# NIRVANALAN/GaussianAnything

Hardware: NVIDIA H100
Metric: 512^2 views/sec @100k Gaussians (surfel raster fwd+bwd) (higher is better)
Workload: dtype f32

## Files before the change

gaussiananything_b200/csrc/raster_bin.cu:

```cuda
#include "raster_common.cuh"
#include "device_once.cuh"

#define SCAN_THREADS 1024
#define SCAN_TILES_PER_THREAD 8
#define SORT_WARP_MAX 512

__global__ void __launch_bounds__(SCAN_THREADS)
scan_tiles_kernel(RasterDims d, RasterWs ws)
{
    __shared__ uint32_t s_warp[32];
    __shared__ uint32_t s_carry;
    __shared__ int s_big;
    const int n = d.NV * d.T;
    if (threadIdx.x == 0) { s_carry = 0; s_big = 0; }
    __syncthreads();
    const int lane = threadIdx.x & 31, warp = threadIdx.x >> 5;
    const uint4 *cnt4 = reinterpret_cast<const uint4 *>(ws.tile_count);
    for (int base = 0; base < n; base += SCAN_THREADS * SCAN_TILES_PER_THREAD) {
        uint32_t v[SCAN_TILES_PER_THREAD];
#pragma unroll
        for (int j = 0; j < SCAN_TILES_PER_THREAD; j++) {
            const int i = base + j * SCAN_THREADS + threadIdx.x;
            v[j] = 0u;
#pragma unroll
            for (int q = 0; q < GA_TILE_REPLICAS / 4; q++) {
                const uint4 c = i < n ? cnt4[(size_t)i * (GA_TILE_REPLICAS / 4) + q] : make_uint4(0u, 0u, 0u, 0u);
                v[j] += ((c.x + c.y) + c.z) + c.w;
            }
        }
        uint32_t excl[SCAN_TILES_PER_THREAD];
#pragma unroll
        for (int j = 0; j < SCAN_TILES_PER_THREAD; j++) {
            if (base + j * SCAN_THREADS >= n) { excl[j] = 0u; continue; }
            if (v[j] > SORT_WARP_MAX) ws.big_tiles[atomicAdd(&s_big, 1)] = (uint32_t)(base + j * SCAN_THREADS + threadIdx.x);
            uint32_t x = v[j];
#pragma unroll
            for (int o = 1; o < 32; o <<= 1) {
                uint32_t y = __shfl_up_sync(0xffffffffu, x, o);
                if (lane >= o) x += y;
            }
            if (lane == 31) s_warp[warp] = x;
            __syncthreads();
            if (warp == 0) {
                uint32_t wv = s_warp[lane], wx = wv;
#pragma unroll
                for (int o = 1; o < 32; o <<= 1) {
                    uint32_t y = __shfl_up_sync(0xffffffffu, wx, o);
                    if (lane >= o) wx += y;
                }
                s_warp[lane] = wx - wv;
            }
            __syncthreads();
            excl[j] = s_carry + s_warp[warp] + x - v[j];
            __syncthreads();
            if (threadIdx.x == SCAN_THREADS - 1) s_carry = excl[j] + v[j];
            __syncthreads();
        }
#pragma unroll
        for (int j = 0; j < SCAN_TILES_PER_THREAD; j++) {
            const int i = base + j * SCAN_THREADS + threadIdx.x;
            if (i >= n) continue;
            ws.tile_start[i] = excl[j];
            uint32_t run = excl[j];
            uint4 *dst = reinterpret_cast<uint4 *>(ws.tile_count) + (size_t)i * (GA_TILE_REPLICAS / 4);
#pragma unroll
            for (int q = 0; q < GA_TILE_REPLICAS / 4; q++) {
                const uint4 c = cnt4[(size_t)i * (GA_TILE_REPLICAS / 4) + q];
                uint4 cur;
                cur.x = run; run += c.x;
                cur.y = run; run += c.y;
                cur.z = run; run += c.z;
                cur.w = run; run += c.w;
                dst[q] = cur;
            }
        }
    }
    __syncthreads();
    if (threadIdx.x == 0) {
        const uint32_t total = s_carry;
        ws.tile_start[n] = total;
        ws.status[0] = (int32_t)total;
        ws.status[1] = ((int64_t)total > d.max_instances) ? 1 : 0;
        ws.status[3] = s_big;
    }
}

__global__ void __launch_bounds__(256)
scatter_kernel(RasterDims d, RasterWs ws)
{
    const int view = blockIdx.y;
    const int i = blockIdx.x * 256 + threadIdx.x;
    if (i >= d.P || ws.status[1]) return;
    const size_t vi = (size_t)view * d.P + i;
    const uint32_t r = ws.rect[vi];
    if (r == 0) return;
    const int x0 = r & 255, y0 = (r >> 8) & 255, x1 = (r >> 16) & 255, y1 = r >> 24;
    const unsigned long long key =
        ((unsigned long long)__float_as_uint(ws.depth[vi]) << 32) | (unsigned long long)(uint32_t)i;
    const int rep = (threadIdx.x >> 5) & (GA_TILE_REPLICAS - 1);
    for (int y = y0; y < y1; y++)
        for (int x = x0; x < x1; x++) {
            const size_t t = (size_t)view * d.T + y * d.gx + x;
            const uint32_t slot = atomicAdd(&ws.tile_count[t * GA_TILE_REPLICAS + rep], 1u);
            ws.keys[slot] = key;
        }
}

__device__ __forceinline__ void block_bitonic_sort(unsigned long long *a, int n)
{
    int n2 = 1;
    while (n2 < n) n2 <<= 1;
    for (int k = 2; k <= n2; k <<= 1) {
        for (int t = threadIdx.x; t < n2 / 2; t += blockDim.x) {
            const int blk = t / (k / 2), off = t % (k / 2);
            const int i = blk * k + off, p = blk * k + k - 1 - off;
            if (p < n) {
                unsigned long long x = a[i], y = a[p];
                if (x > y) { a[i] = y; a[p] = x; }
            }
        }
        __syncthreads();
        for (int j = k / 4; j >= 1; j >>= 1) {
            for (int t = threadIdx.x; t < n2 / 2; t += blockDim.x) {
                const int i = (t / j) * 2 * j + (t % j), p = i + j;
                if (p < n) {
                    unsigned long long x = a[i], y = a[p];
                    if (x > y) { a[i] = y; a[p] = x; }
                }
            }
            __syncthreads();
        }
    }
}

#define SORT_SMEM_KEYS 4096

template <int KPL>
__device__ __forceinline__ void warp_shuffle_stages(unsigned long long (&v)[KPL], int lane, int k, int jstart)
{
#pragma unroll 1
    for (int j = jstart; j >= 1; j >>= 1) {
        const bool lower = (lane & j) == 0;
#pragma unroll
        for (int r = 0; r < KPL; r++) {
            const bool asc = ((((r << 5) | lane) & k) == 0);
            const unsigned long long mine = v[r];
            const unsigned long long other = __shfl_xor_sync(0xffffffffu, mine, j);
            const bool keep_min = (lower == asc);
            v[r] = keep_min ? (mine < other ? mine : other) : (mine > other ? mine : other);
        }
    }
}

template <int KPL>
__device__ __forceinline__ void warp_bitonic_sort(unsigned long long (&v)[KPL], int lane)
{
    constexpr int N = 32 * KPL;
#pragma unroll 1
    for (int k = 2; k <= 32; k <<= 1) warp_shuffle_stages<KPL>(v, lane, k, k >> 1);
#pragma unroll
    for (int k = 64; k <= N; k <<= 1) {
#pragma unroll
        for (int j = k >> 1; j >= 32; j >>= 1) {
            const int jr = j >> 5;
#pragma unroll
            for (int r = 0; r < KPL; r++) {
                if ((r & jr) == 0) {
                    const bool asc = (((r << 5) & k) == 0);
                    unsigned long long a = v[r], b = v[r | jr];
                    const bool sw = asc ? (a > b) : (a < b);
                    v[r] = sw ? b : a;
                    v[r | jr] = sw ? a : b;
                }
            }
        }
        warp_shuffle_stages<KPL>(v, lane, k, 16);
    }
}

template <int KPL>
__device__ __forceinline__ void warp_sort_tile(unsigned long long *gk, uint32_t *gid, int n, int lane)
{
    unsigned long long v[KPL];
#pragma unroll
    for (int r = 0; r < KPL; r++) {
        const int i = r * 32 + lane;
        v[r] = i < n ? gk[i] : 0xffffffffffffffffull;
    }
    warp_bitonic_sort<KPL>(v, lane);
#pragma unroll
    for (int r = 0; r < KPL; r++) {
        const int i = r * 32 + lane;
        if (i < n) {
            gk[i] = v[r];
            gid[i] = (uint32_t)(v[r] & 0xffffffffull);
        }
    }
}

#define SORT_THREADS 256
__global__ void __launch_bounds__(SORT_THREADS, 3)
sort_tiles_kernel(RasterDims d, RasterWs ws, int big_ctas)
{
    __shared__ unsigned long long s_keys[SORT_SMEM_KEYS];
    if (ws.status[1]) return;
    if ((int)blockIdx.x < big_ctas) {
        const int nbig = ws.status[3];
        for (int b = blockIdx.x; b < nbig; b += big_ctas) {
            const uint32_t t = ws.big_tiles[b];
            const uint32_t start = ws.tile_start[t], end = ws.tile_start[t + 1];
            const int n = (int)(end - start);
            unsigned long long *gk = ws.keys + start;
            if (n <= SORT_SMEM_KEYS) {
                for (int i = threadIdx.x; i < n; i += blockDim.x) s_keys[i] = gk[i];
                __syncthreads();
                block_bitonic_sort(s_keys, n);
                for (int i = threadIdx.x; i < n; i += blockDim.x) {
                    const unsigned long long k = s_keys[i];
                    gk[i] = k;
                    ws.ids[start + i] = (uint32_t)(k & 0xffffffffull);
                }
                __syncthreads();
            } else {
                if (threadIdx.x == 0) atomicAdd(&ws.status[2], 1);
                block_bitonic_sort(gk, n);
                for (int i = threadIdx.x; i < n; i += blockDim.x)
                    ws.ids[start + i] = (uint32_t)(gk[i] & 0xffffffffull);
                __syncthreads();
            }
        }
        return;
    }
    const size_t t = (size_t)(blockIdx.x - big_ctas) * (SORT_THREADS / 32) + (threadIdx.x >> 5);
    if (t >= (size_t)d.NV * d.T) return;
    const int lane = threadIdx.x & 31;
    const uint32_t start = ws.tile_start[t], end = ws.tile_start[t + 1];
    const int n = (int)(end - start);
    if (n == 0 || n > SORT_WARP_MAX) return;
    unsigned long long *gk = ws.keys + start;
    uint32_t *gid = ws.ids + start;
    if (n <= 32) warp_sort_tile<1>(gk, gid, n, lane);
    else if (n <= 128) warp_sort_tile<4>(gk, gid, n, lane);
    else if (n <= 256) warp_sort_tile<8>(gk, gid, n, lane);
    else warp_sort_tile<16>(gk, gid, n, lane);
}

cudaError_t ga_launch_binning(const RasterDims &d, const RasterWs &w, cudaStream_t s, int32_t *status_host,
                              cudaEvent_t status_event)
{
    scan_tiles_kernel<<<1, SCAN_THREADS, 0, s>>>(d, w);
    if (status_host) {
        cudaError_t e = cudaMemcpyAsync(status_host, w.status, 4 * sizeof(int32_t), cudaMemcpyDeviceToHost, s);
        if (e != cudaSuccess) return e;
    }
    if (status_event) {
        cudaError_t e = cudaEventRecord(status_event, s);
        if (e != cudaSuccess) return e;
    }
    dim3 grid((d.P + 255) / 256, d.NV);
    scatter_kernel<<<grid, 256, 0, s>>>(d, w);
    const int tiles = d.NV * d.T;
    const int big_ctas = tiles < ga_sm_count() ? tiles : ga_sm_count();
    sort_tiles_kernel<<<big_ctas + (tiles + SORT_THREADS / 32 - 1) / (SORT_THREADS / 32), SORT_THREADS, 0, s>>>(d, w, big_ctas);
    return cudaGetLastError();
}
```

gaussiananything_b200/csrc/raster_render.cu:

```cuda
#include "raster_common.cuh"
#include "device_once.cuh"

#define CHUNK 256

__device__ __forceinline__ float fast_rcp(float x)
{
    float r;
    asm("rcp.approx.ftz.f32 %0, %1;" : "=f"(r) : "f"(x));
    return r;
}
__device__ __forceinline__ float fast_ex2(float x)
{
    float r;
    asm("ex2.approx.ftz.f32 %0, %1;" : "=f"(r) : "f"(x));
    return r;
}
#define GA_M_C0 (GA_FAR_N / (GA_FAR_N - GA_NEAR_N))
#define GA_M_C1 (GA_FAR_N * GA_NEAR_N / (GA_FAR_N - GA_NEAR_N))
#define GA_NEG_HALF_LOG2E (-0.72134752044448170368f)

struct PixelGeom {
    float s0, s1, p2, rho3d, rho2d, dx, dy, depth, G, alpha;
    bool use3d;
};

__device__ __forceinline__ bool eval_pair(const float4 a, const float4 b, const float4 c,
                                          float pfx, float pfy, PixelGeom &o,
                                          float &k0, float &k1, float &k2,
                                          float &l0, float &l1, float &l2)
{
    k0 = pfx * b.z - a.x; k1 = pfx * b.w - a.y; k2 = pfx * c.x - a.z;
    l0 = pfy * b.z - a.w; l1 = pfy * b.w - b.x; l2 = pfy * c.x - b.y;
    const float p0 = k1 * l2 - k2 * l1, p1 = k2 * l0 - k0 * l2, p2 = k0 * l1 - k1 * l0;
    if (p2 == 0.0f) return false;
    const float ip = fast_rcp(p2);
    o.p2 = p2;
    o.s0 = p0 * ip; o.s1 = p1 * ip;
    o.rho3d = o.s0 * o.s0 + o.s1 * o.s1;
    o.dx = c.y - pfx; o.dy = c.z - pfy;
    o.rho2d = GA_FILTER_INV_SQUARE * (o.dx * o.dx + o.dy * o.dy);
    o.use3d = o.rho3d <= o.rho2d;
    const float rho = fminf(o.rho3d, o.rho2d);
    o.depth = o.use3d ? (o.s0 * b.z + o.s1 * b.w) + c.x : c.x;
    if (o.depth < GA_NEAR_N) return false;
    o.G = fast_ex2(rho * GA_NEG_HALF_LOG2E);
    o.alpha = fminf(0.99f, c.w * o.G);
    return o.alpha >= 1.0f / 255.0f;
}

struct TileBox { int x0, y0, w, h; };
__device__ __forceinline__ TileBox clip_box(const float4 bb, int ox, int oy, int xmax, int ymax)
{
    const float x0 = ceilf(fmaxf(bb.x, (float)ox)), x1 = floorf(fminf(bb.y, (float)xmax));
    const float y0 = ceilf(fmaxf(bb.z, (float)oy)), y1 = floorf(fminf(bb.w, (float)ymax));
    if (!(x1 >= x0 && y1 >= y0)) return {0, 0, 0, 0};
    return {(int)x0 - ox, (int)y0 - oy, (int)(x1 - x0) + 1, (int)(y1 - y0) + 1};
}

#define FWD_PAIRS 4096

struct FwdSmem {
    float4 rec[6][CHUNK];
    float2 pair[FWD_PAIRS];
    uint32_t mask[CHUNK / 32][256];
    int base[CHUNK + 1];
    uint32_t box[CHUNK];
    int cnt[CHUNK];
    int wsum[8];
};

template <bool LISTS>
__global__ void __launch_bounds__(256, 3)
render_fwd_kernel(RasterDims d, RasterWs ws, const float *__restrict__ bg,
                  float *__restrict__ out_color, float *__restrict__ out_allmap)
{
    extern __shared__ __align__(16) uint8_t fwd_smem_raw[];
    FwdSmem &sm = *reinterpret_cast<FwdSmem *>(fwd_smem_raw);
    if (ws.status[1]) return;
    const int view = blockIdx.z;
    const int tile = blockIdx.y * d.gx + blockIdx.x;
    const int warp = threadIdx.x >> 5, lane = threadIdx.x & 31;
    const int ox = blockIdx.x * GA_BLOCK_X, oy = blockIdx.y * GA_BLOCK_Y;
    const int lxi = (warp & 1) * 8 + (lane & 7), lyi = (warp >> 1) * 4 + (lane >> 3);
    const int pix_local = lyi * 16 + lxi;
    const int pxi = ox + lxi, pyi = oy + lyi;
    const bool inside = pxi < d.W && pyi < d.H;
    const float oxf = (float)ox, oyf = (float)oy;

    const uint32_t start = ws.tile_start[(size_t)view * d.T + tile];
    const uint32_t end = ws.tile_start[(size_t)view * d.T + tile + 1];
    const int total = (int)(end - start);
    const float *rec_base = ws.rec + (size_t)view * d.P * GA_REC_F;

    bool done = !inside;
    float T = 1.0f, C0 = 0, C1 = 0, C2 = 0, N0 = 0, N1 = 0, N2 = 0;
    float Dacc = 0, M1 = 0, M2 = 0, dist = 0, median_depth = 0;
    int last_contributor = 0, median_contributor = -1;
    int nl = 0;
    uint4 *my_list = nullptr;
    if (LISTS) my_list = ws.lists + ((size_t)view * d.T + tile) * (size_t)d.list_k * 256 + pix_local;

    for (int c0 = 0; c0 < total; c0 += CHUNK) {
        if (__syncthreads_count(done) == 256) break;
        const int cnt = min(CHUNK, total - c0);
        if (LISTS) sm.cnt[threadIdx.x] = 0;
        int npairs = 0;
        if ((int)threadIdx.x < cnt) {
            const uint32_t id = ws.ids[start + c0 + threadIdx.x];
            const float4 *src = reinterpret_cast<const float4 *>(rec_base + (size_t)id * GA_REC_F);
            const float4 a = __ldg(src), b = __ldg(src + 1), c = __ldg(src + 2);
            const float4 nr = __ldg(src + 3), bb = __ldg(src + 4), gb = __ldg(src + 5);
            const float k0 = oxf * b.z - a.x, k1 = oxf * b.w - a.y, k2 = oxf * c.x - a.z;
            const float l0 = oyf * b.z - a.w, l1 = oyf * b.w - b.x, l2 = oyf * c.x - b.y;
            const float Cx = k1 * l2 - k2 * l1, Cy = k2 * l0 - k0 * l2, Cz = k0 * l1 - k1 * l0;
            const float Ax = b.w * l2 - c.x * l1, Ay = c.x * l0 - b.z * l2, Az = b.z * l1 - b.w * l0;
            const float Bx = k1 * c.x - k2 * b.w, By = k2 * b.z - k0 * c.x, Bz = k0 * b.w - k1 * b.z;
            sm.rec[0][threadIdx.x] = make_float4(Cx, Cy, Cz, Ax);
            sm.rec[1][threadIdx.x] = make_float4(Ay, Az, Bx, By);
            sm.rec[2][threadIdx.x] = make_float4(Bz, b.z, b.w, c.x);
            sm.rec[3][threadIdx.x] = make_float4(c.y - oxf, c.z - oyf, c.w, 0.f);
            sm.rec[4][threadIdx.x] = nr;
            sm.rec[5][threadIdx.x] = gb;
            const TileBox q = clip_box(bb, ox, oy, min(ox + 15, d.W - 1), min(oy + 15, d.H - 1));
            npairs = q.w * q.h;
            sm.box[threadIdx.x] = npairs ? (uint32_t)(q.x0 | q.y0 << 4 | q.w << 8 | (65536 / q.w + 1) << 13) : 0u;
        }
        int incl = npairs;
#pragma unroll
        for (int o = 1; o < 32; o <<= 1) {
            const int y = __shfl_up_sync(0xffffffffu, incl, o);
            if (lane >= o) incl += y;
        }
        if (lane == 31) sm.wsum[warp] = incl;
        __syncthreads();
#pragma unroll
        for (int k = 0; k < 8; k++) incl += k < warp ? sm.wsum[k] : 0;
        sm.base[threadIdx.x] = incl - npairs;
        if (threadIdx.x == CHUNK - 1) sm.base[CHUNK] = incl;

        int t0 = 0, base = 0;
        while (t0 < cnt) {
#pragma unroll
            for (int k = 0; k < CHUNK / 32; k++) sm.mask[k][threadIdx.x] = 0u;
            const int t1 = t0 + __syncthreads_count((int)threadIdx.x >= t0 && (int)threadIdx.x < cnt &&
                                                    incl - base <= FWD_PAIRS);
            const int wpairs = sm.base[t1] - base;
            for (int q = threadIdx.x; q < wpairs; q += 256) {
                const int Q = base + q;
                int jj = t0;
#pragma unroll
                for (int step = CHUNK / 2; step > 0; step >>= 1)
                    if (jj + step < t1 && sm.base[jj + step] <= Q) jj += step;
                const uint32_t bx = sm.box[jj];
                const int k = Q - sm.base[jj], w = (bx >> 8) & 31;
                const int ry = (k * (int)(bx >> 13)) >> 16;
                const int lx = (int)(bx & 15) + k - ry * w, ly = (int)((bx >> 4) & 15) + ry;
                const float dxf = (float)lx, dyf = (float)ly;
                const float4 f0 = sm.rec[0][jj], f1 = sm.rec[1][jj], f2 = sm.rec[2][jj], f3 = sm.rec[3][jj];
                const float p0 = f0.x + dxf * f0.w + dyf * f1.z;
                const float p1 = f0.y + dxf * f1.x + dyf * f1.w;
                const float p2 = f0.z + dxf * f1.y + dyf * f2.x;
                const float ip = fast_rcp(p2);
                const float s0 = p0 * ip, s1 = p1 * ip;
                const float rho3d = s0 * s0 + s1 * s1;
                const float ddx = f3.x - dxf, ddy = f3.y - dyf;
                const float rho2d = GA_FILTER_INV_SQUARE * __fmaf_rn(ddx, ddx, __fmul_rn(ddy, ddy));
                const float rho = fminf(rho3d, rho2d);
                const float depth = (rho3d <= rho2d) ? (s0 * f2.y + s1 * f2.z) + f2.w : f2.w;
                const float alpha = fminf(0.99f, f3.z * fast_ex2(rho * GA_NEG_HALF_LOG2E));
                if (p2 != 0.0f && depth >= GA_NEAR_N && alpha >= 1.0f / 255.0f) {
                    sm.pair[q] = make_float2(alpha, depth);
                    atomicOr(&sm.mask[jj >> 5][ly * 16 + lx], 1u << (jj & 31));
                }
            }
            __syncthreads();
            if (!done) {
                int wi = t0 >> 5;
                const int wlast = (t1 - 1) >> 5;
                uint32_t m = sm.mask[wi][pix_local];
                while (true) {
                    while (m == 0u && wi < wlast) m = sm.mask[++wi][pix_local];
                    if (m == 0u) break;
                    const int jj = wi * 32 + __ffs(m) - 1;
                    m &= m - 1;
                    const uint32_t bx = sm.box[jj];
                    const int k = (lyi - (int)((bx >> 4) & 15)) * (int)((bx >> 8) & 31) + (lxi - (int)(bx & 15));
                    const float2 ad = sm.pair[sm.base[jj] - base + k];
                    const float alpha = ad.x, depth = ad.y;
                    const float test_T = T * (1 - alpha);
                    if (test_T < 0.0001f) { done = true; break; }
                    const float4 nr = sm.rec[4][jj], gb = sm.rec[5][jj];
                    const int contributor = c0 + jj + 1;
                    const float w = alpha * T;
                    const float A = 1 - T;
                    const float mm = GA_M_C0 - GA_M_C1 * fast_rcp(depth);
                    dist += (mm * mm * A + M2 - 2 * mm * M1) * w;
                    Dacc += depth * w;
                    M1 += mm * w;
                    M2 += mm * mm * w;
                    if (T > 0.5f) { median_depth = depth; median_contributor = contributor; }
                    N0 += nr.x * w; N1 += nr.y * w; N2 += nr.z * w;
                    C0 += nr.w * w; C1 += gb.x * w; C2 += gb.y * w;
                    T = test_T;
                    last_contributor = contributor;
                    if (LISTS) {
                        atomicAdd(&sm.cnt[jj], 1);
                        if (nl < d.list_k)
                            my_list[(size_t)nl * 256] = make_uint4((uint32_t)(contributor - 1), __float_as_uint(alpha),
                                                                   __float_as_uint(depth), 0u);
                        nl++;
                    }
                }
            }
            t0 = t1;
            if (t0 < cnt) base = sm.base[t0];
            if (__syncthreads_count(done) == 256) break;
        }
        if (LISTS && (int)threadIdx.x < cnt) ws.inst_cnt[start + c0 + threadIdx.x] = (uint32_t)sm.cnt[threadIdx.x];
    }
    if (LISTS) {
        if (inside) ws.n_list[(size_t)view * d.H * d.W + (size_t)pyi * d.W + pxi] = nl;
        if (nl > d.list_k) ws.tile_flag[(size_t)view * d.T + tile] = 1u;
    }
    if (inside) {
        const size_t HW = (size_t)d.H * d.W;
        const size_t pix = (size_t)pyi * d.W + pxi;
        float *fT = ws.final_T + (size_t)view * 3 * HW;
        int32_t *nc = ws.n_contrib + (size_t)view * 2 * HW;
        fT[pix] = T; fT[pix + HW] = M1; fT[pix + 2 * HW] = M2;
        nc[pix] = last_contributor; nc[pix + HW] = median_contributor;
        float *oc = out_color + (size_t)view * 3 * HW;
        oc[pix] = C0 + T * bg[0]; oc[pix + HW] = C1 + T * bg[1]; oc[pix + 2 * HW] = C2 + T * bg[2];
        float *oa = out_allmap + (size_t)view * 7 * HW;
        oa[pix] = Dacc;
        oa[pix + HW] = 1 - T;
        oa[pix + 2 * HW] = N0; oa[pix + 3 * HW] = N1; oa[pix + 4 * HW] = N2;
        oa[pix + 5 * HW] = median_depth;
        oa[pix + 6 * HW] = dist;
    }
}

cudaError_t ga_launch_render_fwd(const RasterDims &d, const RasterWs &w, const float *bg,
                                 float *out_color, float *out_allmap, cudaStream_t s)
{
    static GaPerDevice attr_set;
    if (ga_first_use_on_device(attr_set)) {
        cudaError_t e = cudaFuncSetAttribute(render_fwd_kernel<true>, cudaFuncAttributeMaxDynamicSharedMemorySize,
                                             (int)sizeof(FwdSmem));
        if (e == cudaSuccess)
            e = cudaFuncSetAttribute(render_fwd_kernel<false>, cudaFuncAttributeMaxDynamicSharedMemorySize,
                                     (int)sizeof(FwdSmem));
        if (e != cudaSuccess) return e;
    }
    dim3 grid(d.gx, d.gy, d.NV);
    if (d.list_k > 0) render_fwd_kernel<true><<<grid, 256, sizeof(FwdSmem), s>>>(d, w, bg, out_color, out_allmap);
    else render_fwd_kernel<false><<<grid, 256, sizeof(FwdSmem), s>>>(d, w, bg, out_color, out_allmap);
    return cudaGetLastError();
}

#define BWD_RECORDS 4096
#define BWD_TPI 2

struct BwdSmem {
    float4 rec[6][CHUNK];
    uint4 recs[BWD_RECORDS];
    float4 up[3][256];
    uint32_t id[CHUNK];
    int off[CHUNK];
    int cnt[CHUNK];
    int bin[64];
    uint16_t perm[CHUNK];
    int wsum[8];
    int maxc, m;
};

template <int TPI>
__device__ __forceinline__ void reduce_scatter18(const float (&g)[GA_GRAD_F], int lane, float *__restrict__ dst)
{
    int off = 0, size = 9;
    float a9[10];
    {
        const bool u = lane & (TPI >> 1);
#pragma unroll
        for (int i = 0; i < 9; i++) {
            const float keep = u ? g[9 + i] : g[i], send = u ? g[i] : g[9 + i];
            a9[i] = keep + __shfl_xor_sync(0xffffffffu, send, TPI >> 1);
        }
        a9[9] = 0.f;
        off += u ? 9 : 0;
    }
    if constexpr (TPI == 2) {
#pragma unroll
        for (int i = 0; i < 9; i++)
            if (a9[i] != 0.f) atomicAdd(dst + off + i, a9[i]);
        return;
    } else {
        float b5[6];
        {
            const bool u = lane & (TPI >> 2);
#pragma unroll
            for (int i = 0; i < 5; i++) {
                const float keep = u ? a9[5 + i] : a9[i], send = u ? a9[i] : a9[5 + i];
                b5[i] = keep + __shfl_xor_sync(0xffffffffu, send, TPI >> 2);
            }
            b5[5] = 0.f;
            off += u ? 5 : 0; size = u ? 4 : 5;
        }
        if constexpr (TPI == 4) {
#pragma unroll
            for (int i = 0; i < 5; i++)
                if (i < size && b5[i] != 0.f) atomicAdd(dst + off + i, b5[i]);
            return;
        } else {
            float c3[4];
            {
                const bool u = lane & (TPI >> 3);
#pragma unroll
                for (int i = 0; i < 3; i++) {
                    const float keep = u ? b5[3 + i] : b5[i], send = u ? b5[i] : b5[3 + i];
                    c3[i] = keep + __shfl_xor_sync(0xffffffffu, send, TPI >> 3);
                }
                c3[3] = 0.f;
                off += u ? 3 : 0; size = u ? size - 3 : 3;
            }
            if constexpr (TPI == 8) {
#pragma unroll
                for (int i = 0; i < 3; i++)
                    if (i < size && c3[i] != 0.f) atomicAdd(dst + off + i, c3[i]);
                return;
            } else {
                const bool u = lane & (TPI >> 4);
                float d2[2];
#pragma unroll
                for (int i = 0; i < 2; i++) {
                    const float keep = u ? c3[2 + i] : c3[i], send = u ? c3[i] : c3[2 + i];
                    d2[i] = keep + __shfl_xor_sync(0xffffffffu, send, TPI >> 4);
                }
                off += u ? 2 : 0; size = u ? max(size - 2, 0) : min(size, 2);
#pragma unroll
                for (int i = 0; i < 2; i++)
                    if (i < size && d2[i] != 0.f) atomicAdd(dst + off + i, d2[i]);
            }
        }
    }
}

__device__ __forceinline__ int clipped_box_area(const float4 bb, int ox, int oy)
{
    const TileBox q = clip_box(bb, ox, oy, ox + 15, oy + 15);
    return q.w * q.h;
}

template <bool LISTS>
__device__ __forceinline__ void bwd_tile(const RasterDims &d, const RasterWs &ws, BwdSmem &sm, const float *__restrict__ bg,
                                         const float *__restrict__ dL_dcolor, const float *__restrict__ dL_dallmap,
                                         float *__restrict__ grad_acc)
{
    const int view = blockIdx.z;
    const int tile = blockIdx.y * d.gx + blockIdx.x;
    const int warp = threadIdx.x >> 5, lane = threadIdx.x & 31;
    const int ox = blockIdx.x * GA_BLOCK_X, oy = blockIdx.y * GA_BLOCK_Y;
    const int lx0 = (warp & 1) * 8, ly0 = (warp >> 1) * 4;
    const int lxi = lx0 + (lane & 7), lyi = ly0 + (lane >> 3);
    const int pxi = ox + lxi, pyi = oy + lyi;
    const int pix_local = lyi * 16 + lxi;
    const bool inside = pxi < d.W && pyi < d.H;
    const float pfx = (float)pxi, pfy = (float)pyi;

    const uint32_t start = ws.tile_start[(size_t)view * d.T + tile];
    const size_t HW = (size_t)d.H * d.W;
    const size_t pix = inside ? (size_t)pyi * d.W + pxi : 0;
    const float *fT = ws.final_T + (size_t)view * 3 * HW;
    const int32_t *nc = ws.n_contrib + (size_t)view * 2 * HW;
    const float *rec_base = ws.rec + (size_t)view * d.P * GA_REC_F;
    float *acc_base = grad_acc + (size_t)view * d.P * GA_GRAD_F;

    const float T_final = inside ? fT[pix] : 0.f;
    float T = T_final;
    const int last_contributor = inside ? nc[pix] : 0;
    const int median_contributor = inside ? nc[pix + HW] : 0;
    float bg_dot_dpixel = 0.f;
    {
        float4 u0 = make_float4(0.f, 0.f, 0.f, 0.f), u1 = u0, u2 = u0;
        if (inside) {
            const float *gc = dL_dcolor + (size_t)view * 3 * HW;
            const float *ga = dL_dallmap + (size_t)view * 7 * HW;
            u0 = make_float4(gc[pix], gc[pix + HW], gc[pix + 2 * HW], ga[pix + 2 * HW]);
            u1 = make_float4(ga[pix + 3 * HW], ga[pix + 4 * HW], ga[pix], ga[pix + HW]);
            u2 = make_float4(ga[pix + 6 * HW], ga[pix + 5 * HW], fT[pix + HW], fT[pix + 2 * HW]);
        }
        sm.up[0][pix_local] = u0;
        sm.up[1][pix_local] = u1;
        sm.up[2][pix_local] = u2;
        bg_dot_dpixel = bg[0] * u0.x + bg[1] * u0.y + bg[2] * u0.z;
    }
    const float final_A = 1 - T_final;
    float last_alpha = 0, v_last = 0, v_acc = 0, last_dL_dT = 0;

    const uint4 *my_list = nullptr;
    int kk = -1;
    if (LISTS) {
        my_list = ws.lists + ((size_t)view * d.T + tile) * (size_t)d.list_k * 256 + pix_local;
        kk = (inside ? ws.n_list[(size_t)view * HW + pix] : 0) - 1;
#pragma unroll
        for (int q = 0; q < 8; q++)
            if (kk >= q) asm volatile("prefetch.global.L2 [%0];" ::"l"(my_list + (size_t)(kk - q) * 256));
    }

    if (threadIdx.x == 0) sm.maxc = 0;
    __syncthreads();
    {
        int mc = last_contributor;
#pragma unroll
        for (int o = 16; o > 0; o >>= 1) mc = max(mc, __shfl_xor_sync(0xffffffffu, mc, o));
        if (lane == 0) atomicMax(&sm.maxc, mc);
    }
    __syncthreads();
    const int total = sm.maxc;

    for (int hi = total; hi > 0; hi -= CHUNK) {
        const int cnt = min(CHUNK, hi);
        int bound = 0;
        if ((int)threadIdx.x < cnt) {
            const int pos = hi - 1 - (int)threadIdx.x;
            const uint32_t id = ws.ids[start + pos];
            sm.id[threadIdx.x] = id;
            const float4 *src = reinterpret_cast<const float4 *>(rec_base + (size_t)id * GA_REC_F);
            float4 q[6];
#pragma unroll
            for (int k = 0; k < 6; k++) { q[k] = __ldg(src + k); sm.rec[k][threadIdx.x] = q[k]; }
            bound = LISTS ? (int)ws.inst_cnt[start + pos] : clipped_box_area(q[4], ox, oy);
        }
        int incl = bound;
#pragma unroll
        for (int o = 1; o < 32; o <<= 1) {
            const int y = __shfl_up_sync(0xffffffffu, incl, o);
            if (lane >= o) incl += y;
        }
        if (lane == 31) sm.wsum[warp] = incl;
        __syncthreads();
#pragma unroll
        for (int k = 0; k < 8; k++) incl += k < warp ? sm.wsum[k] : 0;
        sm.off[threadIdx.x] = incl - bound;
        sm.cnt[threadIdx.x] = 0;

        int t0 = 0, base = 0;
        while (t0 < cnt) {
            if (threadIdx.x < 64) sm.bin[threadIdx.x] = 0;
            const int t1 = t0 + __syncthreads_count((int)threadIdx.x >= t0 && (int)threadIdx.x < cnt &&
                                                    incl - base <= BWD_RECORDS);

            auto contribute = [&](const int jj, const int contributor, const float alpha, const float c_d) {
                const float4 nr = sm.rec[3][jj], gb = sm.rec[5][jj];
                const float4 u0 = sm.up[0][pix_local], u1 = sm.up[1][pix_local], u2 = sm.up[2][pix_local];
                const float dL_ddepth = u1.z, dL_dreg = u2.x, final_D = u2.z, final_D2 = u2.w;
                const float inv1ma = fast_rcp(1.f - alpha);
                T = T * inv1ma;
                const float w = alpha * T;
                float dL_dz = 0.0f;
                const float inv_cd = fast_rcp(c_d);
                const float m_d = GA_M_C0 - GA_M_C1 * inv_cd;
                const float dmd_dd = GA_M_C1 * inv_cd * inv_cd;
                if (contributor == median_contributor - 1) dL_dz += u2.y;
                const float dL_dweight = (final_D2 + m_d * m_d * final_A - 2 * m_d * final_D) * dL_dreg;
                const float dL_dmd = 2.0f * (T * alpha) * (m_d * final_A - final_D) * dL_dreg;
                dL_dz += dL_dmd * dmd_dd;
                const float v = ((nr.w * u0.x + gb.x * u0.y) + (gb.y * u0.z + c_d * dL_ddepth)) +
                                ((nr.x * u0.w + nr.y * u1.x) + (nr.z * u1.y + u1.w));
                v_acc = last_alpha * v_last + (1.f - last_alpha) * v_acc;
                v_last = v;
                float dL_dalpha = (v - v_acc) + (dL_dweight - last_dL_dT);
                last_dL_dT = dL_dweight * alpha + (1 - alpha) * last_dL_dT;
                dL_dalpha *= T;
                last_alpha = alpha;
                dL_dalpha += (-T_final * inv1ma) * bg_dot_dpixel;
                dL_dz += w * dL_ddepth;
                const int slot = atomicAdd(&sm.cnt[jj], 1);
                sm.recs[sm.off[jj] - base + slot] =
                    make_uint4((uint32_t)pix_local, __float_as_uint(dL_dalpha), __float_as_uint(dL_dz), __float_as_uint(w));
            };
            if constexpr (LISTS) {
                const int pos_lo = hi - t1;
                uint4 e = make_uint4(0u, 0u, 0u, 0u), e1 = e, e2 = e;
                if (kk >= 0) e = __ldg(my_list + (size_t)kk * 256);
                if (kk >= 1) e1 = __ldg(my_list + (size_t)(kk - 1) * 256);
                if (kk >= 2) e2 = __ldg(my_list + (size_t)(kk - 2) * 256);
                while (true) {
                    const bool active = kk >= 0 && (int)e.x >= pos_lo;
                    if (!__any_sync(0xffffffffu, active)) break;
                    if (active) {
                        const uint4 cur = e;
                        e = e1; e1 = e2;
                        if (kk >= 3) e2 = __ldg(my_list + (size_t)(kk - 3) * 256);
                        if (kk >= 8) asm volatile("prefetch.global.L2 [%0];" ::"l"(my_list + (size_t)(kk - 8) * 256));
                        kk--;
                        contribute(hi - 1 - (int)cur.x, (int)cur.x, __uint_as_float(cur.y), __uint_as_float(cur.z));
                    }
                }
            } else {
                const float bx_lo = (float)(ox + lx0), bx_hi = (float)(ox + lx0 + 7);
                const float by_lo = (float)(oy + ly0), by_hi = (float)(oy + ly0 + 3);
                for (int sb = t0; sb < t1; sb += 32) {
                    bool hit = false;
                    if (sb + lane < t1) {
                        const float4 bb = sm.rec[4][sb + lane];
                        hit = !(bb.y < bx_lo || bb.x > bx_hi || bb.w < by_lo || bb.z > by_hi);
                    }
                    unsigned mask = __ballot_sync(0xffffffffu, hit);
                    unsigned mine = 0;
                    while (mask) {
                        const int b = __ffs(mask) - 1;
                        mask &= mask - 1;
                        const float4 bb = sm.rec[4][sb + b];
                        if (pfx >= bb.x && pfx <= bb.y && pfy >= bb.z && pfy <= bb.w && (hi - 1 - (sb + b)) < last_contributor)
                            mine |= 1u << b;
                    }
                    if (!inside) mine = 0;
                    while (__any_sync(0xffffffffu, mine != 0)) {
                        const bool active = mine != 0;
                        const int bsel = active ? __ffs(mine) - 1 : 0;
                        mine &= mine - 1;
                        const int jj = sb + bsel;
                        const float4 a = sm.rec[0][jj], b = sm.rec[1][jj], c = sm.rec[2][jj];
                        PixelGeom pg;
                        float k0, k1, k2, l0, l1, l2;
                        const bool ok = active && eval_pair(a, b, c, pfx, pfy, pg, k0, k1, k2, l0, l1, l2);
                        if (ok) contribute(jj, hi - 1 - jj, pg.alpha, pg.depth);
                    }
                }
            }
            __syncthreads();

            const int myc = ((int)threadIdx.x >= t0 && (int)threadIdx.x < t1) ? sm.cnt[threadIdx.x] : 0;
            if (myc > 0) atomicAdd(&sm.bin[min(myc, 63)], 1);
            __syncthreads();
            if (threadIdx.x < 32) {
                const int hi_bin = 63 - 2 * (int)threadIdx.x, lo_bin = hi_bin - 1;
                const int vh = sm.bin[hi_bin], vl = lo_bin >= 1 ? sm.bin[lo_bin] : 0;
                int x = vh + vl;
#pragma unroll
                for (int o = 1; o < 32; o <<= 1) {
                    const int y = __shfl_up_sync(0xffffffffu, x, o);
                    if ((int)threadIdx.x >= o) x += y;
                }
                const int excl = x - (vh + vl);
                sm.bin[hi_bin] = excl;
                if (lo_bin >= 1) sm.bin[lo_bin] = excl + vh;
                if (threadIdx.x == 31) sm.m = x;
            }
            __syncthreads();
            if (myc > 0) sm.perm[atomicAdd(&sm.bin[min(myc, 63)], 1)] = (uint16_t)threadIdx.x;
            __syncthreads();
            const int m = sm.m, sub = threadIdx.x % BWD_TPI;
            for (int b0 = 0; b0 < m; b0 += 256 / BWD_TPI) {
                const int slot = b0 + (int)threadIdx.x / BWD_TPI;
                const int jj = slot < m ? (int)sm.perm[slot] : 0;
                const int n = slot < m ? sm.cnt[jj] : 0;
                float g[GA_GRAD_F];
#pragma unroll
                for (int f = 0; f < GA_GRAD_F; f++) g[f] = 0.f;
                if (n > 0) {
                    const float4 a = sm.rec[0][jj], b = sm.rec[1][jj], c = sm.rec[2][jj];
                    const float opa = c.w;
                    const uint4 *lst = sm.recs + (sm.off[jj] - base);
                    for (int r = sub; r < n; r += BWD_TPI) {
                        const uint4 rc = lst[r];
                        const int p = (int)rc.x;
                        const float dL_dalpha = __uint_as_float(rc.y), dL_dz = __uint_as_float(rc.z), w = __uint_as_float(rc.w);
                        const float qx = (float)(ox + (p & 15)), qy = (float)(oy + (p >> 4));
                        PixelGeom pg;
                        float k0, k1, k2, l0, l1, l2;
                        eval_pair(a, b, c, qx, qy, pg, k0, k1, k2, l0, l1, l2);
                        const float G = pg.G;
                        const float dL_dG = opa * dL_dalpha;
                        if (pg.use3d) {
                            const float dL_ds0 = dL_dG * -G * pg.s0 + dL_dz * b.z;
                            const float dL_ds1 = dL_dG * -G * pg.s1 + dL_dz * b.w;
                            const float ip = fast_rcp(pg.p2);
                            const float q0 = dL_ds0 * ip, q1 = dL_ds1 * ip;
                            const float q2 = -(q0 * pg.s0 + q1 * pg.s1);
                            const float dk0 = l1 * q2 - l2 * q1, dk1 = l2 * q0 - l0 * q2, dk2 = l0 * q1 - l1 * q0;
                            const float dl0 = q1 * k2 - q2 * k1, dl1 = q2 * k0 - q0 * k2, dl2 = q0 * k1 - q1 * k0;
                            g[0] -= dk0; g[1] -= dk1; g[2] -= dk2;
                            g[3] -= dl0; g[4] -= dl1; g[5] -= dl2;
                            g[6] += qx * dk0 + qy * dl0 + dL_dz * pg.s0;
                            g[7] += qx * dk1 + qy * dl1 + dL_dz * pg.s1;
                            g[8] += qx * dk2 + qy * dl2 + dL_dz;
                        } else {
                            g[9] += dL_dG * (-G * GA_FILTER_INV_SQUARE * pg.dx);
                            g[10] += dL_dG * (-G * GA_FILTER_INV_SQUARE * pg.dy);
                            g[8] += dL_dz;
                        }
                        g[14] += G * dL_dalpha;
                        const float4 ua = sm.up[0][p], ub = sm.up[1][p];
                        g[15] += w * ua.x; g[16] += w * ua.y; g[17] += w * ua.z;
                        g[11] += w * ua.w; g[12] += w * ub.x; g[13] += w * ub.y;
                    }
                }
                if (__any_sync(0xffffffffu, n > 0))
                    reduce_scatter18<BWD_TPI>(g, lane, acc_base + (size_t)(n > 0 ? sm.id[jj] : 0) * GA_GRAD_F);
            }
            t0 = t1;
            if (t0 < cnt) base = sm.off[t0];
            __syncthreads();
        }
    }
}

__global__ void __launch_bounds__(256, 2)
render_bwd_kernel(RasterDims d, RasterWs ws, const float *__restrict__ bg, const float *__restrict__ dL_dcolor,
                  const float *__restrict__ dL_dallmap, float *__restrict__ grad_acc)
{
    extern __shared__ __align__(16) uint8_t bwd_smem_raw[];
    BwdSmem &sm = *reinterpret_cast<BwdSmem *>(bwd_smem_raw);
    if (ws.status[1]) return;
    if (d.list_k > 0 && ws.tile_flag[(size_t)blockIdx.z * d.T + blockIdx.y * d.gx + blockIdx.x] == 0)
        bwd_tile<true>(d, ws, sm, bg, dL_dcolor, dL_dallmap, grad_acc);
    else
        bwd_tile<false>(d, ws, sm, bg, dL_dcolor, dL_dallmap, grad_acc);
}

cudaError_t ga_launch_render_bwd(const RasterDims &d, const RasterWs &w, const float *bg,
                                 const float *dL_dcolor, const float *dL_dallmap, float *grad_acc, cudaStream_t s)
{
    static GaPerDevice attr_set;
    if (ga_first_use_on_device(attr_set)) {
        cudaError_t e = cudaFuncSetAttribute(render_bwd_kernel, cudaFuncAttributeMaxDynamicSharedMemorySize,
                                             (int)sizeof(BwdSmem));
        if (e != cudaSuccess) return e;
    }
    dim3 grid(d.gx, d.gy, d.NV);
    render_bwd_kernel<<<grid, 256, sizeof(BwdSmem), s>>>(d, w, bg, dL_dcolor, dL_dallmap, grad_acc);
    return cudaGetLastError();
}
```

Baseline: 6343.

## Fuse per-tile depth sort into the forward render kernel

Removes the standalone sort_tiles_kernel and instead sorts each tile's keys inside render_fwd_kernel. It uses the shared pair buffer as scratch: a warp bitonic sort per segment, then a rank-based merge across warps, with a block bitonic fallback for larger tiles. While loading keys it issues L2 prefetches of the Gaussian records, and the first chunk reads ids straight from shared memory. This drops a kernel launch and a global key pass, but the render kernel may run short of registers, and the sort now runs on the render critical path.

New measurement: 6614, median of 6. 1.04x the previous value.

```diff
diff --git a/gaussiananything_b200/csrc/raster_bin.cu b/gaussiananything_b200/csrc/raster_bin.cu
--- a/gaussiananything_b200/csrc/raster_bin.cu
+++ b/gaussiananything_b200/csrc/raster_bin.cu
@@ -1,9 +1,8 @@
 #include "raster_common.cuh"
-#include "device_once.cuh"
 
 #define SCAN_THREADS 1024
 #define SCAN_TILES_PER_THREAD 8
-#define SORT_WARP_MAX 512
+#define BIG_TILE_INSTANCES 512
 
 __global__ void __launch_bounds__(SCAN_THREADS)
 scan_tiles_kernel(RasterDims d, RasterWs ws)
@@ -32,7 +31,7 @@
 #pragma unroll
         for (int j = 0; j < SCAN_TILES_PER_THREAD; j++) {
             if (base + j * SCAN_THREADS >= n) { excl[j] = 0u; continue; }
-            if (v[j] > SORT_WARP_MAX) ws.big_tiles[atomicAdd(&s_big, 1)] = (uint32_t)(base + j * SCAN_THREADS + threadIdx.x);
+            if (v[j] > BIG_TILE_INSTANCES) ws.big_tiles[atomicAdd(&s_big, 1)] = (uint32_t)(base + j * SCAN_THREADS + threadIdx.x);
             uint32_t x = v[j];
 #pragma unroll
             for (int o = 1; o < 32; o <<= 1) {
@@ -106,145 +105,6 @@
         }
 }
 
-__device__ __forceinline__ void block_bitonic_sort(unsigned long long *a, int n)
-{
-    int n2 = 1;
-    while (n2 < n) n2 <<= 1;
-    for (int k = 2; k <= n2; k <<= 1) {
-        for (int t = threadIdx.x; t < n2 / 2; t += blockDim.x) {
-            const int blk = t / (k / 2), off = t % (k / 2);
-            const int i = blk * k + off, p = blk * k + k - 1 - off;
-            if (p < n) {
-                unsigned long long x = a[i], y = a[p];
-                if (x > y) { a[i] = y; a[p] = x; }
-            }
-        }
-        __syncthreads();
-        for (int j = k / 4; j >= 1; j >>= 1) {
-            for (int t = threadIdx.x; t < n2 / 2; t += blockDim.x) {
-                const int i = (t / j) * 2 * j + (t % j), p = i + j;
-                if (p < n) {
-                    unsigned long long x = a[i], y = a[p];
-                    if (x > y) { a[i] = y; a[p] = x; }
-                }
-            }
-            __syncthreads();
-        }
-    }
-}
-
-#define SORT_SMEM_KEYS 4096
-
-template <int KPL>
-__device__ __forceinline__ void warp_shuffle_stages(unsigned long long (&v)[KPL], int lane, int k, int jstart)
-{
-#pragma unroll 1
-    for (int j = jstart; j >= 1; j >>= 1) {
-        const bool lower = (lane & j) == 0;
-#pragma unroll
-        for (int r = 0; r < KPL; r++) {
-            const bool asc = ((((r << 5) | lane) & k) == 0);
-            const unsigned long long mine = v[r];
-            const unsigned long long other = __shfl_xor_sync(0xffffffffu, mine, j);
-            const bool keep_min = (lower == asc);
-            v[r] = keep_min ? (mine < other ? mine : other) : (mine > other ? mine : other);
-        }
-    }
-}
-
-template <int KPL>
-__device__ __forceinline__ void warp_bitonic_sort(unsigned long long (&v)[KPL], int lane)
-{
-    constexpr int N = 32 * KPL;
-#pragma unroll 1
-    for (int k = 2; k <= 32; k <<= 1) warp_shuffle_stages<KPL>(v, lane, k, k >> 1);
-#pragma unroll
-    for (int k = 64; k <= N; k <<= 1) {
-#pragma unroll
-        for (int j = k >> 1; j >= 32; j >>= 1) {
-            const int jr = j >> 5;
-#pragma unroll
-            for (int r = 0; r < KPL; r++) {
-                if ((r & jr) == 0) {
-                    const bool asc = (((r << 5) & k) == 0);
-                    unsigned long long a = v[r], b = v[r | jr];
-                    const bool sw = asc ? (a > b) : (a < b);
-                    v[r] = sw ? b : a;
-                    v[r | jr] = sw ? a : b;
-                }
-            }
-        }
-        warp_shuffle_stages<KPL>(v, lane, k, 16);
-    }
-}
-
-template <int KPL>
-__device__ __forceinline__ void warp_sort_tile(unsigned long long *gk, uint32_t *gid, int n, int lane)
-{
-    unsigned long long v[KPL];
-#pragma unroll
-    for (int r = 0; r < KPL; r++) {
-        const int i = r * 32 + lane;
-        v[r] = i < n ? gk[i] : 0xffffffffffffffffull;
-    }
-    warp_bitonic_sort<KPL>(v, lane);
-#pragma unroll
-    for (int r = 0; r < KPL; r++) {
-        const int i = r * 32 + lane;
-        if (i < n) {
-            gk[i] = v[r];
-            gid[i] = (uint32_t)(v[r] & 0xffffffffull);
-        }
-    }
-}
-
-#define SORT_THREADS 256
-__global__ void __launch_bounds__(SORT_THREADS, 3)
-sort_tiles_kernel(RasterDims d, RasterWs ws, int big_ctas)
-{
-    __shared__ unsigned long long s_keys[SORT_SMEM_KEYS];
-    if (ws.status[1]) return;
-    if ((int)blockIdx.x < big_ctas) {
-        const int nbig = ws.status[3];
-        for (int b = blockIdx.x; b < nbig; b += big_ctas) {
-            const uint32_t t = ws.big_tiles[b];
-            const uint32_t start = ws.tile_start[t], end = ws.tile_start[t + 1];
-            const int n = (int)(end - start);
-            unsigned long long *gk = ws.keys + start;
-            if (n <= SORT_SMEM_KEYS) {
-                for (int i = threadIdx.x; i < n; i += blockDim.x) s_keys[i] = gk[i];
-                __syncthreads();
-                block_bitonic_sort(s_keys, n);
-                for (int i = threadIdx.x; i < n; i += blockDim.x) {
-                    const unsigned long long k = s_keys[i];
-                    gk[i] = k;
-                    ws.ids[start + i] = (uint32_t)(k & 0xffffffffull);
-                }
-                __syncthreads();
-            } else {
-                if (threadIdx.x == 0) atomicAdd(&ws.status[2], 1);
-                block_bitonic_sort(gk, n);
-                for (int i = threadIdx.x; i < n; i += blockDim.x)
-                    ws.ids[start + i] = (uint32_t)(gk[i] & 0xffffffffull);
-                __syncthreads();
-            }
-        }
-        return;
-    }
-    const size_t t = (size_t)(blockIdx.x - big_ctas) * (SORT_THREADS / 32) + (threadIdx.x >> 5);
-    if (t >= (size_t)d.NV * d.T) return;
-    const int lane = threadIdx.x & 31;
-    const uint32_t start = ws.tile_start[t], end = ws.tile_start[t + 1];
-    const int n = (int)(end - start);
-    if (n == 0 || n > SORT_WARP_MAX) return;
-    unsigned long long *gk = ws.keys + start;
-    uint32_t *gid = ws.ids + start;
-    if (n <= 32) warp_sort_tile<1>(gk, gid, n, lane);
-    else if (n <= 128) warp_sort_tile<4>(gk, gid, n, lane);
-    else if (n <= 256) warp_sort_tile<8>(gk, gid, n, lane);
-    else warp_sort_tile<16>(gk, gid, n, lane);
-}
-
 cudaError_t ga_launch_binning(const RasterDims &d, const RasterWs &w, cudaStream_t s, int32_t *status_host,
                               cudaEvent_t status_event)
 {
@@ -259,8 +119,5 @@
     }
     dim3 grid((d.P + 255) / 256, d.NV);
     scatter_kernel<<<grid, 256, 0, s>>>(d, w);
-    const int tiles = d.NV * d.T;
-    const int big_ctas = tiles < ga_sm_count() ? tiles : ga_sm_count();
-    sort_tiles_kernel<<<big_ctas + (tiles + SORT_THREADS / 32 - 1) / (SORT_THREADS / 32), SORT_THREADS, 0, s>>>(d, w, big_ctas);
     return cudaGetLastError();
 }
diff --git a/gaussiananything_b200/csrc/raster_render.cu b/gaussiananything_b200/csrc/raster_render.cu
--- a/gaussiananything_b200/csrc/raster_render.cu
+++ b/gaussiananything_b200/csrc/raster_render.cu
@@ -69,6 +69,145 @@
     int wsum[8];
 };
 
+__device__ __forceinline__ void block_bitonic_sort(unsigned long long *a, int n)
+{
+    int n2 = 1;
+    while (n2 < n) n2 <<= 1;
+    for (int k = 2; k <= n2; k <<= 1) {
+        for (int t = threadIdx.x; t < n2 / 2; t += blockDim.x) {
+            const int blk = t / (k / 2), off = t % (k / 2);
+            const int i = blk * k + off, p = blk * k + k - 1 - off;
+            if (p < n) {
+                unsigned long long x = a[i], y = a[p];
+                if (x > y) { a[i] = y; a[p] = x; }
+            }
+        }
+        __syncthreads();
+        for (int j = k / 4; j >= 1; j >>= 1) {
+            for (int t = threadIdx.x; t < n2 / 2; t += blockDim.x) {
+                const int i = (t / j) * 2 * j + (t % j), p = i + j;
+                if (p < n) {
+                    unsigned long long x = a[i], y = a[p];
+                    if (x > y) { a[i] = y; a[p] = x; }
+                }
+            }
+            __syncthreads();
+        }
+    }
+}
+
+template <int KPL>
+__device__ __forceinline__ void warp_shuffle_stages(unsigned long long (&v)[KPL], int lane, int k, int jstart)
+{
+#pragma unroll
+    for (int j = jstart; j >= 1; j >>= 1) {
+        const bool lower = (lane & j) == 0;
+#pragma unroll
+        for (int r = 0; r < KPL; r++) {
+            const bool asc = ((((r << 5) | lane) & k) == 0);
+            const unsigned long long mine = v[r];
+            const unsigned long long other = __shfl_xor_sync(0xffffffffu, mine, j);
+            const bool keep_min = (lower == asc);
+            v[r] = ((other < mine) == keep_min) ? other : mine;
+        }
+    }
+}
+
+template <int KPL>
+__device__ __forceinline__ void warp_bitonic_sort(unsigned long long (&v)[KPL], int lane)
+{
+    constexpr int N = 32 * KPL;
+#pragma unroll
+    for (int k = 2; k <= 32; k <<= 1) warp_shuffle_stages<KPL>(v, lane, k, k >> 1);
+#pragma unroll
+    for (int k = 64; k <= N; k <<= 1) {
+#pragma unroll
+        for (int j = k >> 1; j >= 32; j >>= 1) {
+            const int jr = j >> 5;
+#pragma unroll
+            for (int r = 0; r < KPL; r++) {
+                if ((r & jr) == 0) {
+                    const bool asc = (((r << 5) & k) == 0);
+                    unsigned long long a = v[r], b = v[r | jr];
+                    const bool sw = asc ? (a > b) : (a < b);
+                    v[r] = sw ? b : a;
+                    v[r | jr] = sw ? a : b;
+                }
+            }
+        }
+        warp_shuffle_stages<KPL>(v, lane, k, 16);
+    }
+}
+
+template <int KPL>
+__device__ __forceinline__ void block_merge_sort(const unsigned long long *src, unsigned long long *a, int n,
+                                                 const float *rec)
+{
+    constexpr int SEG = 32 * KPL;
+    const int warp = threadIdx.x >> 5, lane = threadIdx.x & 31;
+    const int nseg = (n + SEG - 1) / SEG;
+    unsigned long long v[KPL];
+    int rank[KPL];
+    if (warp < nseg) {
+#pragma unroll
+        for (int r = 0; r < KPL; r++) {
+            const int i = warp * SEG + r * 32 + lane;
+            v[r] = i < n ? src[i] : ~0ull;
+            if (i < n) asm volatile("prefetch.global.L2 [%0];" ::"l"(rec + (size_t)(uint32_t)v[r] * GA_REC_F));
+        }
+        warp_bitonic_sort<KPL>(v, lane);
+#pragma unroll
+        for (int r = 0; r < KPL; r++) a[warp * SEG + r * 32 + lane] = v[r];
+    }
+    __syncthreads();
+    if (warp < nseg) {
+#pragma unroll
+        for (int r = 0; r < KPL; r++) rank[r] = r * 32 + lane;
+        for (int sg = 0; sg < nseg; sg++) {
+            if (sg == warp) continue;
+            const unsigned long long *run = a + sg * SEG;
+#pragma unroll
+            for (int r = 0; r < KPL; r++) {
+                int lo = 0;
+#pragma unroll
+                for (int step = SEG / 2; step >= 1; step >>= 1)
+                    if (run[lo + step - 1] < v[r]) lo += step;
+                rank[r] += lo + (run[lo] < v[r] ? 1 : 0);
+            }
+        }
+    }
+    __syncthreads();
+    if (warp < nseg) {
+#pragma unroll
+        for (int r = 0; r < KPL; r++)
+            if (warp * SEG + r * 32 + lane < n) a[rank[r]] = v[r];
+    }
+    __syncthreads();
+}
+
+__device__ __forceinline__ void sort_tile(const RasterWs &ws, uint32_t start, int n, unsigned long long *s, const float *rec)
+{
+    unsigned long long *gk = ws.keys + start;
+    if (n > FWD_PAIRS) {
+        if (threadIdx.x == 0) atomicAdd(&ws.status[2], 1);
+        block_bitonic_sort(gk, n);
+        for (int i = threadIdx.x; i < n; i += 256) ws.ids[start + i] = (uint32_t)(gk[i] & 0xffffffffull);
+        return;
+    }
+    if (n <= 256) block_merge_sort<1>(gk, s, n, rec);
+    else if (n <= 512) block_merge_sort<2>(gk, s, n, rec);
+    else {
+        for (int i = threadIdx.x; i < n; i += 256) s[i] = gk[i];
+        __syncthreads();
+        block_bitonic_sort(s, n);
+    }
+    for (int i = threadIdx.x; i < n; i += 256) {
+        const unsigned long long k = s[i];
+        gk[i] = k;
+        ws.ids[start + i] = (uint32_t)(k & 0xffffffffull);
+    }
+}
+
 template <bool LISTS>
 __global__ void __launch_bounds__(256, 3)
 render_fwd_kernel(RasterDims d, RasterWs ws, const float *__restrict__ bg,
@@ -100,13 +239,17 @@
     uint4 *my_list = nullptr;
     if (LISTS) my_list = ws.lists + ((size_t)view * d.T + tile) * (size_t)d.list_k * 256 + pix_local;
 
+    const unsigned long long *skeys = reinterpret_cast<const unsigned long long *>(sm.pair);
+    sort_tile(ws, start, total, reinterpret_cast<unsigned long long *>(sm.pair), rec_base);
+
     for (int c0 = 0; c0 < total; c0 += CHUNK) {
         if (__syncthreads_count(done) == 256) break;
         const int cnt = min(CHUNK, total - c0);
         if (LISTS) sm.cnt[threadIdx.x] = 0;
         int npairs = 0;
         if ((int)threadIdx.x < cnt) {
-            const uint32_t id = ws.ids[start + c0 + threadIdx.x];
+            const uint32_t id = (c0 == 0 && total <= FWD_PAIRS) ? (uint32_t)(skeys[threadIdx.x] & 0xffffffffull)
+                                                                : ws.ids[start + c0 + threadIdx.x];
             const float4 *src = reinterpret_cast<const float4 *>(rec_base + (size_t)id * GA_REC_F);
             const float4 a = __ldg(src), b = __ldg(src + 1), c = __ldg(src + 2);
             const float4 nr = __ldg(src + 3), bb = __ldg(src + 4), gb = __ldg(src + 5);
```
